# apache/datafusion-ballista

Measured on NVIDIA B200. Metric: tpch_q1_rows_per_sec, higher is better.
Workload: dtype decimal128/i128

## Files before the change

### datafusion-ballista_b200/csrc/device/kernels.cu

```cuda
#include <cuda_runtime.h>
#include <stdint.h>

#include "../common/hash.hpp"
#include "../common/tpch_gen.hpp"
#include "kernels.h"

namespace b200 {

typedef __int128 i128;
typedef unsigned __int128 u128;

static inline int grid_for(int64_t n, int block, int per_thread = 1) {
  int64_t g = (n + (int64_t)block * per_thread - 1) / ((int64_t)block * per_thread);
  if (g < 1) g = 1;
  if (g > 148 * 16) g = 148 * 16;
  return (int)g;
}

__global__ void agg_table_init_kernel(AggTable T, AccKinds kinds) {
  for (unsigned long long i = blockIdx.x * (unsigned long long)blockDim.x + threadIdx.x; i < T.cap; i += (unsigned long long)gridDim.x * blockDim.x) {
    T.hash[i] = 0;
    T.state[i] = 0;
    T.lock[i] = 0;
    for (int a = 0; a < kinds.n; a++) {
// ... 26 lines not shown
    case PH_I8:
    case PH_U8:
    case PH_BOOL8: ((int8_t*)data)[pos] = (int8_t)v; break;
    case PH_I16:
    case PH_U16: ((int16_t*)data)[pos] = (int16_t)v; break;
    case PH_I32:
    case PH_U32: ((int32_t*)data)[pos] = (int32_t)v; break;
    default: ((long long*)data)[pos] = v;
  }
}

__global__ void agg_extract_kernel(AggTable T, AggExtractArgs A) {
  for (unsigned long long s = blockIdx.x * (unsigned long long)blockDim.x + threadIdx.x; s < T.cap; s += (unsigned long long)gridDim.x * blockDim.x) {
    if (T.state[s] != 2) continue;
    unsigned long long pos = atomicAdd(A.counter, 1ull);
    for (int j = 0; j < A.n_out; j++) {
      const AggOut& o = A.out[j];
      switch (o.kind) {
        case AO_KEY: {
          unsigned long long w0 = T.keys[((unsigned long long)o.a * T.cap + s) * 2 + 0];
          unsigned long long w1 = T.keys[((unsigned long long)o.a * T.cap + s) * 2 + 1];
          unsigned char v = T.key_valid[(unsigned long long)o.a * T.cap + s];
          if (o.phys == PH_DEC128 || o.phys == PH_STRVIEW) ((ulonglong2*)o.data)[pos] = make_ulonglong2(w0, w1);
          else if (o.phys == PH_F64) ((unsigned long long*)o.data)[pos] = w0;
          else if (o.phys == PH_F32) ((float*)o.data)[pos] = (float)__longlong_as_double((long long)w0);
          else store_typed_i64(o.data, o.phys, pos, (long long)w0);
          if (o.valid) o.valid[pos] = v;
          break;
        }
        case AO_KEY_PACKED: {
// ... 786 lines not shown
```

### datafusion-ballista_b200/csrc/device/kernels.h

```cpp
#pragma once
#include <cuda_runtime.h>
#include <stdint.h>

#include "program.h"

namespace b200 {

cudaError_t launch_pipeline(const Program& P, int reg_groups, int grid, int block, size_t smem, cudaStream_t st);
cudaError_t launch_fused_pipeline(const Program& P, const FusedSpec& F, FusedShape shape, int reg_groups, int grid, int block, size_t smem, cudaStream_t st,
                                  int* is_static);
bool fused_rows_ok(const Program& P, int grid, int block, int rows_per_thread);
bool pipeline_add_only(const Program& P, int grid, int block);

struct AccKinds {
  uint8_t kind[VM_MAX_ACC];
  int n;
};
void launch_agg_table_init(const AggTable& T, const AccKinds& kinds, cudaStream_t st);

enum AggOutKind : uint8_t {
  AO_KEY = 0,
  AO_ACC_I128,
  AO_ACC_I64,
  AO_ACC_F64,
// ... 5 lines not shown
};
struct AggOut {
  void* data;
  uint8_t* valid;
  void* aux;
  uint8_t kind;
  uint8_t a, b;
  uint8_t phys;
  int32_t imm;
};
struct AggExtractArgs {
  AggOut out[VM_MAX_OUT];
  int n_out;
  int n_keys;
  unsigned long long* counter;
  unsigned int* error;
};
void launch_agg_extract(const AggTable& T, const AggExtractArgs& A, cudaStream_t st);

void launch_scan_u32_to_u64(const uint32_t* in, uint64_t* out, int64_t n, uint64_t* scratch , cudaStream_t st);
void launch_histogram_u32(const uint32_t* ids, int64_t n, uint32_t n_bins, unsigned long long* counts, cudaStream_t st);
uint64_t launch_partition_dest_stable(const uint32_t* ids, int64_t n, uint32_t n_bins, uint32_t* dest, uint64_t* keys_a, uint32_t* vals_a, uint64_t* keys_b,
                                      uint32_t* vals_b, uint32_t* hist_scratch, uint64_t* scan_scratch, cudaStream_t st);
void launch_scatter_fixed(const void* in, void* out, const uint32_t* dest, int64_t n, int width, cudaStream_t st);
void launch_gather_fixed(const void* in, const uint8_t* valid_in, void* out, uint8_t* valid_out, const int64_t* idx, int64_t n, int width, cudaStream_t st);
static const int GATHER_MAX_COLS = 32;
struct GatherCol {
  const void* in;
  const uint8_t* valid_in;
  void* out;
// ... 212 lines not shown
```

### datafusion-ballista_b200/csrc/host/engine.cpp

```cpp
#include <sched.h>
#include <sys/stat.h>

#include <algorithm>
#include <atomic>
#include <cctype>
#include <chrono>
#include <cmath>
#include <cstdio>
#include <map>
#include <mutex>
#include <functional>
#include <set>

#include "../common/arrow_host.hpp"
#include "../common/tpch_gen.hpp"
#include "../device/kernels.h"
#include "host_pool.hpp"
#include "lower.hpp"
#include "nccl_dyn.hpp"
#include "../common/plan_proto.hpp"
#include "../common/plan_dump.hpp"
#include "parquet_meta.hpp"
#include "arrow_ipc.hpp"

// ... 34 lines not shown
  int sm_count = 148;
  cudaStream_t own_stream = nullptr;
  cudaStream_t stream = nullptr;
  std::mutex mu;
  std::map<std::string, std::map<int, DevBatchPtr>> tables;
  std::map<ShuffleKey, std::vector<Piece>> shuffle;
  std::map<ShuffleKey, DevBatchPtr> packed_cache;
  std::atomic<uint64_t> launches{0};
  std::atomic<uint64_t> n_fused{0}, n_fused_static{0}, n_vm{0}, n_groupby{0}, n_groupby_pf{0}, n_fastfilter{0};
  int64_t batch_size = 8192;
  std::map<std::string, std::string> config;
  std::map<std::string, int> agg_hint;
  uint64_t pf_bucket_slots = (uint64_t)1 << 19;
  int64_t pf_min_rows = (int64_t)1 << 22;
  std::map<std::string, uint64_t> agg_groups;
  void* pinned_stage = nullptr;
  std::unique_ptr<HostPool> pool;
  std::mutex ingest_mu;
  struct NarrowSlot {
    void* pinned = nullptr;
    void* dev = nullptr;
    cudaEvent_t done = nullptr;
    bool used = false;
    size_t bytes = 0;
  } nslot[4];
  int64_t ingest_chunk_rows = (int64_t)1 << 22;
  int ingest_slots = 3;
  bool kernel_timing = false;
  struct KernelSample { std::string name; cudaEvent_t e0, e1; uint64_t bytes; };
  std::vector<KernelSample> ksamples;
  struct KernelStat { double ms = 0; uint64_t launches = 0, bytes = 0; };
  std::map<std::string, KernelStat> kstats;
  ncclComm_t comm = nullptr;
  std::mutex comm_mu;
  uint64_t exch_sent_bytes = 0, exch_recv_bytes = 0;
  size_t win_config_bytes = 0;
  uint8_t* win_local = nullptr;
  size_t win_bytes = 0, win_used = 0;
  std::vector<uint8_t*> win_peer;
  uint64_t fused_exchanges = 0;
  std::mutex export_mu;
  uint8_t* export_arena = nullptr;
  std::atomic<uint64_t> narrowed_bytes_saved{0};
};

struct b200_stage {
  b200_engine* eng = nullptr;
  std::string job_id;
  int64_t stage_id = 0;
  PlanPtr plan;
  std::string fingerprint;
  std::vector<OpMetrics> metrics;
  std::map<const PlanNode*, int> metric_index;
};

#define NCCL_CHECK(expr)                                                                                              \
  do {                                                                                                                \
    ncclResult_t _r = (expr);                                                                                         \
    if (_r != 0) throw EngineError(B200_ERR_CUDA, std::string("NCCL error: ") + NcclApi::get().GetErrorString(_r) + " at " + __FILE__ + ":" + std::to_string(__LINE__)); \
  } while (0)

static void release_window(b200_engine* e);
static void setup_window(b200_engine* e);

namespace {

struct TaskCtx {
  uint8_t* arena = nullptr;
  size_t pos = 0;
  bool drained = true;
  std::vector<std::function<void()>> checks;
};
static const size_t TASK_ARENA_BYTES = (size_t)1 << 16;
inline TaskCtx& task_ctx() {
  static thread_local TaskCtx t;
  if (!t.arena && cudaHostAlloc((void**)&t.arena, TASK_ARENA_BYTES, cudaHostAllocDefault) != cudaSuccess) t.arena = nullptr;
  return t;
}

struct Exec {
  b200_engine* e;
  b200_stage* s;
  const volatile int32_t* cancel;
  cudaStream_t st() const { return e->stream; }
  void check_cancel() const {
    if (cancel && *cancel) throw EngineError(B200_ERR_CANCELLED, "task cancelled");
  }
  void count(uint64_t n = 1) const { e->launches.fetch_add(n, std::memory_order_relaxed); }
  OpMetrics* m(const PlanNode* n) const {
    if (!s) return nullptr;
    auto it = s->metric_index.find(n);
    return it == s->metric_index.end() ? nullptr : &s->metrics[(size_t)it->second];
  }
  const void* fetch_bytes(const void* dptr, size_t bytes) const {
    TaskCtx& t = task_ctx();
    if (!t.arena) throw EngineError(B200_ERR_OOM, "pinned read-back arena unavailable");
    if (t.drained) {
      t.pos = 0;
// ... 21 lines not shown
      t.pos = 0;
      t.drained = false;
      at = 0;
      if (bytes > TASK_ARENA_BYTES) throw EngineError(B200_ERR_INVALID, "staging request larger than the arena");
    }
    t.pos = at + bytes;
    return t.arena + at;
  }
  template <class T>
  const T* fetch(const void* dptr) const {
    return (const T*)fetch_bytes(dptr, sizeof(T));
  }
  void defer(std::function<void()> fn) const { task_ctx().checks.push_back(std::move(fn)); }
  void sync() const {
    TaskCtx& t = task_ctx();
    cudaError_t se = cudaStreamSynchronize(st());
    t.drained = true;
    std::vector<std::function<void()>> cs;
    cs.swap(t.checks);
    CUDA_CHECK(se);
    for (auto& c : cs) c();
    check_cancel();
  }
  static void abandon() {
    TaskCtx& t = task_ctx();
    t.checks.clear();
    t.drained = true;
  }
  template <class T>
  T get(const void* dptr) const {
    const T* p = fetch<T>(dptr);
    sync();
    return *p;
  }
};

struct KernelTimer {
// ... 526 lines not shown
      CUDA_CHECK(cudaMemsetAsync(cnt->ptr, 0, 8, st));
      launch_bytes_to_bitmap(c.valid, (uint8_t*)bm->ptr, n, (unsigned long long*)cnt->ptr, st);
      x.count();
      h.validity.resize((size_t)(n + 7) / 8);
      CUDA_CHECK(cudaMemcpyAsync(h.validity.data(), bm->ptr, h.validity.size(), cudaMemcpyDeviceToHost, st));
      h.null_count = (int64_t)x.get<unsigned long long>(cnt->ptr);
      if (h.null_count == 0) h.validity.clear();
    }
    if (c.type.id == TypeId::Bool) {
      h.data.assign((size_t)(n + 7) / 8, 0);
      if (n) {
        DevPtr bm = dev_alloc((size_t)(n + 7) / 8 + 16, st);
        launch_bytes_to_bitmap(c.data, (uint8_t*)bm->ptr, n, nullptr, st);
        x.count();
        CUDA_CHECK(cudaMemcpyAsync(h.data.data(), bm->ptr, h.data.size(), cudaMemcpyDeviceToHost, st));
        CUDA_CHECK(cudaStreamSynchronize(st));
      }
    } else if (c.type.id == TypeId::Utf8) {
      DevColumn u = c.phys == PH_STRVIEW ? as_utf8(x, c) : c;
      h.data.resize((size_t)(n + 1) * 4);
      CUDA_CHECK(cudaMemcpyAsync(h.data.data(), u.data, h.data.size(), cudaMemcpyDeviceToHost, st));
      CUDA_CHECK(cudaStreamSynchronize(st));
      int32_t* off = (int32_t*)h.data.data();
      int32_t first = off[0], last = off[n];
      h.extra.resize((size_t)(last - first));
      if (last > first) CUDA_CHECK(cudaMemcpyAsync(h.extra.data(), u.chars + first, h.extra.size(), cudaMemcpyDeviceToHost, st));
      CUDA_CHECK(cudaStreamSynchronize(st));
      for (int64_t i = 0; i <= n; i++) off[i] -= first;
    } else {
      h.data.resize((size_t)n * c.width());
      if (n) CUDA_CHECK(cudaMemcpyAsync(h.data.data(), c.data, h.data.size(), cudaMemcpyDeviceToHost, st));
      CUDA_CHECK(cudaStreamSynchronize(st));
    }
    hcs.push_back(std::move(h));
  }
  return hcs;
}

void export_batch(const Exec& x, const DevBatch& b, int64_t r0, int64_t r1, ArrowArray* out, ArrowSchema* out_schema) {
  std::vector<HostCol> hcs = download_batch(x, b, r0, r1);
  export_record_batch(std::move(hcs), r1 - r0, out, out_schema);
}

struct RunOutcome {
  RunStatus status;
  float ms = 0;
};

struct FusedPlan {
  FusedSpec spec;
  FusedShape shape;
  int block = 0;
  size_t smem = 0;
};

static void throw_run_error(unsigned int error) {
  if (error == 1) throw EngineError(B200_ERR_EXECUTION, "Arithmetic overflow");
  if (error == 2) throw EngineError(B200_ERR_EXECUTION, "Divide by zero");
  if (error) throw EngineError(B200_ERR_EXECUTION, "execution error in expression");
}

// ... 156 lines not shown
  CUDA_CHECK(cudaEventRecord(e1, x.st()));
  x.count();
  RunOutcome o;
  const RunStatus* hs = x.fetch<RunStatus>(dstat->ptr);
  const unsigned int* he = extra_fetch ? x.fetch<unsigned int>(extra_fetch) : nullptr;
  if (!wait) {
    x.defer([hs, e0, e1, met, dstat, tstate]() {
      float ms = 0;
      cudaEventElapsedTime(&ms, e0, e1);
      cudaEventDestroy(e0);
      cudaEventDestroy(e1);
      if (met) met->elapsed_ns += (uint64_t)(ms * 1e6);
      throw_run_error(hs->error);
    });
    memset(&o.status, 0, sizeof o.status);
    return o;
  }
  try {
    x.sync();
  } catch (...) {
    cudaEventDestroy(e0);
    cudaEventDestroy(e1);
    throw;
  }
  o.status = *hs;
  if (he && extra_out) *extra_out = *he;
  cudaEventElapsedTime(&o.ms, e0, e1);
  cudaEventDestroy(e0);
  cudaEventDestroy(e1);
  if (met) met->elapsed_ns += (uint64_t)(o.ms * 1e6);
// ... 719 lines not shown
    S.out_data[j] = oc.data;
  }
  S.n_out = P.n_out;
  S.n_rows = P.n_rows;
  return true;
}

struct TableMem {
  AggTable T;
  std::vector<DevPtr> keep;
};

TableMem alloc_table(const Exec& x, uint64_t cap, int n_keys, const std::vector<AccDesc>& accs) {
  TableMem tm;
  memset(&tm.T, 0, sizeof tm.T);
  auto A = [&](size_t bytes) {
    DevPtr p = dev_alloc(bytes, x.st());
    tm.keep.push_back(p);
    return p->ptr;
  };
  tm.T.cap = cap;
  tm.T.hash = (unsigned long long*)A(cap * 8);
  tm.T.state = (unsigned int*)A(cap * 4);
  tm.T.lock = (unsigned int*)A(cap * 4);
  tm.T.keys = (unsigned long long*)A(std::max<size_t>(1, (size_t)n_keys) * cap * 16);
  tm.T.key_valid = (unsigned char*)A(std::max<size_t>(1, (size_t)n_keys) * cap);
  tm.T.acc = (unsigned long long*)A(std::max<size_t>(1, accs.size()) * cap * 16);
  tm.T.n_groups = (unsigned int*)A(16);
  AccKinds k;
  memset(&k, 0, sizeof k);
  k.n = (int)accs.size();
  for (size_t i = 0; i < accs.size(); i++) k.kind[i] = accs[i].kind;
  launch_agg_table_init(tm.T, k, x.st());
  x.count();
  return tm;
}

typedef std::function<std::unique_ptr<PipelineBuilder>()> BuilderFactory;

DevBatchPtr run_aggregate(const Exec& x, const BuilderFactory& make_pb, const PlanNode& node, const DevBatchPtr& src, OpMetrics* met) {
  const int n_keys = (int)node.group_by.size();
  if (n_keys > VM_MAX_KEYS) throw EngineError(B200_ERR_UNSUPPORTED, "too many group-by columns");
  int pack_mode = 0;
  {
    bool any_str = false, all_narrow = n_keys > 0;
    for (auto& g : node.group_by) {
      any_str |= g.expr->type.id == TypeId::Utf8;
      all_narrow &= narrowable(g.expr->type);
    }
    if (n_keys == 2 && all_narrow) pack_mode = 2;
    else if (any_str) pack_mode = 1;
  }
  int node_idx = -1;
  if (x.s) {
    auto it = x.s->metric_index.find(&node);
    if (it != x.s->metric_index.end()) node_idx = it->second;
  }
  const std::string hint_key = (x.s ? x.s->fingerprint : std::string("?")) + "#" + std::to_string(node_idx);
  int level = 0;
  bool had_hint = false;
  uint64_t groups_hint = 0;
  {
    std::lock_guard<std::mutex> g(x.e->mu);
    auto it = x.e->agg_hint.find(hint_key);
    if (it != x.e->agg_hint.end()) {
      level = it->second / 4;
      pack_mode = std::min(pack_mode, it->second % 4);
      had_hint = true;
      auto ig = x.e->agg_groups.find(hint_key);
      if (ig != x.e->agg_groups.end()) groups_hint = ig->second;
    }
  }
  const int hinted_level = had_hint ? level : -1;
  bool sampled = false;
  std::unique_ptr<PipelineBuilder> pbp;
  AggLowered L;
  TableMem tm;
  RunOutcome ro;
  unsigned int n_groups = 0;
  bool gb_bailed = false, pf_off = false;
  for (;;) {
    x.check_cancel();
    ScopeTimer t_iter("  agg: lower+alloc+launch+sync");
    pbp = make_pb();
    PipelineBuilder& pb = *pbp;
    L = AggLowered();
    lower_aggregate(pb, node, L, pack_mode);
    Program& P = pb.prog;
    P.n_keys = (uint8_t)n_keys;
    P.n_acc = (uint8_t)L.accs.size();
    for (int k = 0; k < n_keys; k++) P.keys[k] = pb.resolve(L.keys[(size_t)k]);
    for (size_t a = 0; a < L.accs.size(); a++) P.acc[a] = L.accs[a];
    memset(&P.key_hash, 0, sizeof P.key_hash);
    P.keys_all_i64 = L.fast ? 1 : 0;
    if (n_keys) {
      if (L.fast) {
// ... 45 lines not shown
        RunOutcome so = launch_program(x, pb, 0, nullptr, true, nullptr, stm.T.n_groups, &seen, &probe);
        if (!so.status.pack_overflow && (so.status.overflow || seen > (unsigned)VM_REG_GROUPS)) {
          level = (so.status.overflow || (int64_t)seen * 2 > sample_rows) ? 3 : 2;
          continue;
        }
      }
      P.table = tm.T;
    }
    FusedPlan fspec;
    const bool use_fused = level == 0 && match_fused(P, fspec);
    GroupBySpec gspec;
    const bool use_gb = level > 0 && !gb_bailed && match_groupby(P, gspec);
    gspec.pf_K = pf_off ? -1 : 0;
    {
      ScopeTimer t_l("    agg: launch_program (incl. sync)");
      ro = launch_program(x, pb, reg_groups, use_fused ? &fspec : nullptr, true, met, tm.T.n_groups, &n_groups, use_gb ? &gspec : nullptr);
    }
    if (met) met->launches += 2;
    if (ro.status.pack_overflow && use_gb) {
      gb_bailed = true;
      continue;
    }
    if (ro.status.pack_overflow) {
      pack_mode = pack_mode == 2 ? 1 : 0;
      continue;
    }
    if (!ro.status.overflow) break;
    if (level > 0 && cap >= next_pow2((uint64_t)std::max<int64_t>(src->n, 1) * 2)) {
      if (use_gb && !pf_off) {
        pf_off = true;
        continue;
      }
      throw EngineError(B200_ERR_EXECUTION, "aggregate hash table overflow");
    }
    level++;
  }
  {
    int learnt = level;
    if (level > 0) {
      learnt = 1;
      while (learnt < 7 && ((uint64_t)1 << (12 + 4 * learnt)) < (uint64_t)n_groups * 2) learnt++;
    }
    std::lock_guard<std::mutex> g(x.e->mu);
    x.e->agg_hint[hint_key] = learnt * 4 + pack_mode;
    uint64_t& gh = x.e->agg_groups[hint_key];
    gh = std::max<uint64_t>(gh, n_groups);
  }
  PipelineBuilder& pb = *pbp;
  ScopeTimer t_ex("  agg: extract");
  auto out = std::make_shared<DevBatch>();
  out->n = n_groups;
  AggExtractArgs A;
  memset(&A, 0, sizeof A);
  if (L.outs.size() > (size_t)VM_MAX_OUT) throw EngineError(B200_ERR_UNSUPPORTED, "too many aggregate output columns");
  A.n_out = (int)L.outs.size();
  A.n_keys = n_keys;
  DevPtr counter = dev_alloc(16, x.st());
  CUDA_CHECK(cudaMemsetAsync(counter->ptr, 0, 16, x.st()));
  A.counter = (unsigned long long*)counter->ptr;
  A.error = (unsigned int*)((uint8_t*)counter->ptr + 8);
  uint64_t wbytes = 0;
  for (size_t j = 0; j < L.outs.size(); j++) {
    const auto& r = L.outs[j];
    DevColumn oc = make_out_column(r.name, r.type, r.phys, n_groups, r.with_valid, x.st());
    oc.n = n_groups;
    if (r.key_idx >= 0) {
      for (auto& k : L.keys[(size_t)r.key_idx].keep) oc.keep.push_back(k);
      if (r.phys == PH_STRVIEW) {
        for (auto& sc : src->cols)
          for (auto& k : sc.keep) oc.keep.push_back(k);
        for (auto& k : pb.keep) oc.keep.push_back(k);
      }
    }
    AggOut& o = A.out[j];
    o.data = (void*)oc.data;
    o.valid = (uint8_t*)oc.valid;
    o.aux = nullptr;
    if (r.kind == AO_KEY_PACKED) {
      DevPtr ch = dev_alloc((size_t)std::max<unsigned int>(n_groups, 1) * 8, x.st());
      o.aux = ch->ptr;
      oc.keep.push_back(ch);
    }
    o.kind = r.kind;
    o.a = r.a;
    o.b = r.b;
    o.phys = r.phys;
    o.imm = r.imm;
    wbytes += (uint64_t)oc.width() * n_groups;
    out->cols.push_back(oc);
  }
  launch_agg_extract(tm.T, A, x.st());
  x.count();
  {
    const unsigned int* herr = x.fetch<unsigned int>(A.error);
    x.defer([herr, counter]() {
      if (*herr) throw EngineError(B200_ERR_EXECUTION, "Arithmetic overflow");
    });
  }
  for (size_t c = 0; c < out->cols.size() && c < node.schema.size(); c++) out->cols[c].name = node.schema[c].name;
  if (met) {
    met->bytes_read += source_bytes(pb);
    met->bytes_written += wbytes;
    met->input_rows += (uint64_t)src->n;
  }
  return out;
}

struct Runner {
  Exec x;
  std::string job;
// ... 7 lines not shown
        return it->second.empty() ? 0 : it->second.rbegin()->first + 1;
      }
      case PlanNode::ShuffleReader: {
        std::lock_guard<std::mutex> g(x.e->mu);
        int mx = 0;
        for (auto& kv : x.e->shuffle)
          if (kv.first.job == job && kv.first.stage == n.reader_stage_id) mx = std::max(mx, (int)kv.first.part + 1);
        return mx;
      }
      case PlanNode::SortPreservingMerge: return 1;
      case PlanNode::Passthrough:
        if (n.op_name == "CoalescePartitionsExec") return 1;
        return n_partitions(*n.children[0]);
      case PlanNode::HashJoin: return n_partitions(*n.children[1]);
      default: return n_partitions(*n.children[0]);
    }
  }

  DevBatchPtr concat(const std::vector<DevBatchPtr>& parts, const Schema& schema) {
    std::vector<std::pair<DevBatchPtr, std::pair<int64_t, int64_t>>> v;
    for (auto& p : parts) v.push_back({p, {0, p->n}});
    return concat_slices(v, schema);
  }

  DevBatchPtr concat_slices(const std::vector<std::pair<DevBatchPtr, std::pair<int64_t, int64_t>>>& parts, const Schema& schema) {
    auto out = std::make_shared<DevBatch>();
    int64_t total = 0;
    for (auto& p : parts) total += p.second.second - p.second.first;
    out->n = total;
    if (parts.size() == 1) {
// ... 179 lines not shown
          const int64_t keep = std::min<int64_t>(all->n, n.fetch);
          out = std::make_shared<DevBatch>();
          out->n = keep;
          for (auto& c : all->cols) out->cols.push_back(slice_column(c, 0, keep));
          break;
        }
        out = with_chain(n, part, false, [&](const BuilderFactory& mk, DevBatchPtr& src) {
          auto pb = mk();
          return run_materialize(x, *pb, named_cols(*pb, n.schema), src, met);
        });
        break;
      }
      case PlanNode::Aggregate: {
        const PlanNode& child = *n.children[0];
        bool all = (n.agg_mode == AggMode::Final || n.agg_mode == AggMode::Single) && part == 0 && n_partitions(child) > 1;
        out = with_chain(child, part, all, [&](const BuilderFactory& mk, DevBatchPtr& src) { return run_aggregate(x, mk, n, src, met); });
        break;
      }
      case PlanNode::HashJoin:
        out = exec_join(n, part, met);
        if (!n.sort_keys.empty()) out = do_sort(n.sort_keys, -1, out, met);
        break;
      case PlanNode::Sort: {
        DevBatchPtr in = exec(*n.children[0], part);
        out = do_sort(n.sort_keys, n.fetch, in, met);
        break;
      }
      case PlanNode::SortPreservingMerge: {
        DevBatchPtr in = exec_all(*n.children[0]);
        out = do_sort(n.sort_keys, n.fetch, in, met);
        break;
      }
      case PlanNode::Passthrough:
        out = (n.op_name == "CoalescePartitionsExec") ? exec_all(*n.children[0]) : exec(*n.children[0], part);
        break;
      case PlanNode::Limit: {
        DevBatchPtr in = (n.op_name == "GlobalLimitExec") ? exec_all(*n.children[0]) : exec(*n.children[0], part);
        int64_t r0 = std::min<int64_t>(std::max<int64_t>(0, n.skip), in->n);
        int64_t r1 = n.fetch >= 0 ? std::min<int64_t>(in->n, r0 + n.fetch) : in->n;
        out = std::make_shared<DevBatch>();
        out->n = r1 - r0;
        for (auto& c : in->cols) out->cols.push_back(slice_column(c, r0, r1));
        break;
      }
// ... 103 lines not shown
          radix_sort_pairs_u64((uint64_t*)ka->ptr, (uint32_t*)vb->ptr, (uint64_t*)kb->ptr, (uint32_t*)va->ptr, n, (uint32_t*)hist->ptr, (uint64_t*)scan->ptr, x.st(), &in_a, &ln);
          perm = in_a ? (uint32_t*)vb->ptr : (uint32_t*)va->ptr;
        }
        x.count(ln);
        (void)perm_alt;
      }
    }
    int64_t m = fetch >= 0 ? std::min<int64_t>(fetch, n) : n;
    DevPtr idx = dev_alloc((size_t)std::max<int64_t>(m, 1) * 8, x.st());
    launch_u32_to_i64(perm, (int64_t*)idx->ptr, m, x.st());
    x.count();
    DevBatch proj;
    proj.n = n;
    for (size_t c = 0; c < n_in_cols; c++) proj.cols.push_back(in->cols[c]);
    DevBatchPtr out = gather_batch(x, proj, (const int64_t*)idx->ptr, m, false);
    CUDA_CHECK(cudaStreamSynchronize(x.st()));
    if (met) {
      met->elapsed_ns += (uint64_t)std::chrono::duration_cast<std::chrono::nanoseconds>(std::chrono::steady_clock::now() - t0).count();
      met->input_rows += (uint64_t)n;
    }
    return out;
  }

  struct Mixed {
    std::vector<DevColumn> cols;
    int64_t n = 0;
  };
  Mixed materialize_mixed(PipelineBuilder& pb, const std::vector<ColRef>& outs, const DevBatchPtr& src, OpMetrics* met) {
    Mixed m;
    const bool filters = program_filters(pb.prog);
    std::vector<int> direct(outs.size(), -1);
// ... 309 lines not shown
  }

  uint64_t slice_bytes(const DevBatch& b, int64_t rows, const std::vector<int64_t>& chars_bytes) {
    uint64_t t = 0;
    size_t si = 0;
    for (auto& c : b.cols) {
      if (c.type.id == TypeId::Bool) t += (uint64_t)(rows + 7) / 8;
      else if (c.type.id == TypeId::Utf8) t += 4ull * (uint64_t)(rows + 1) + (uint64_t)chars_bytes[si++];
      else t += (uint64_t)c.width() * (uint64_t)rows;
    }
    return t;
  }

  std::vector<int64_t> string_bytes(const DevBatch& b) {
    std::vector<int64_t> out;
    PartStrCols sc;
    sc.n = 0;
    std::vector<size_t> unknown;
    for (auto& c : b.cols) {
      if (c.type.id != TypeId::Utf8) continue;
      if (c.phys == PH_UTF8 && c.chars_bytes >= 0) {
        out.push_back(c.chars_bytes);
        continue;
      }
      out.push_back(-1);
      if (b.n == 0) {
        out.back() = 0;
        continue;
      }
      if (sc.n == PART_MAX_STR_COLS) throw EngineError(B200_ERR_UNSUPPORTED, "more than 16 string columns in one shuffle output");
      sc.c[sc.n++] = PartStrCol{c.data, c.valid, c.phys == PH_STRVIEW ? 1 : 0, 0};
      unknown.push_back(out.size() - 1);
    }
    if (sc.n) {
      DevPtr acc = dev_alloc((size_t)(1 + sc.n) * 8, x.st());
      CUDA_CHECK(cudaMemsetAsync(acc->ptr, 0, (size_t)(1 + sc.n) * 8, x.st()));
      PidSrc none;
      memset(&none, 0, sizeof none);
      CUDA_CHECK(launch_partition_hist(none, b.n, 1, nullptr, (unsigned long long*)acc->ptr, sc, (unsigned long long*)acc->ptr + 1, x.st()));
      x.count();
      const unsigned long long* h = (const unsigned long long*)x.fetch_bytes((const unsigned long long*)acc->ptr + 1, (size_t)sc.n * 8);
      x.sync();
      for (size_t k = 0; k < unknown.size(); k++) out[unknown[k]] = (int64_t)h[k];
    }
    return out;
  }

  struct FusedExchange {
    bool done = false;
    uint64_t sent = 0, recvd = 0;
  };

  bool scatter_to_owners(const PlanNode& root, int input_partition, const std::vector<DevColumn>& pay, const PidSrc& pid, int64_t n, uint32_t P,
                         uint32_t n_tiles, const DevPtr& mat, const DevPtr& tile_hist, uint64_t row_bytes, FusedExchange* fx,
                         std::vector<b200_shuffle_write_partition>& res, OpMetrics* met) {
    b200_engine* e = x.e;
    NcclApi& N = NcclApi::get();
    const int W = e->world, me = e->rank;
    const size_t mrow = (size_t)P + 3;
    const size_t ncols = pay.size();
// ... 186 lines not shown
    auto nbatches = [&](uint64_t rows) { return (rows + (uint64_t)bs - 1) / (uint64_t)bs; };
    std::vector<b200_shuffle_write_partition> res;
    const bool single = root.n_out_partitions == 1;
    if (root.n_out_partitions == 0 || single) {
      DevBatchPtr in = exec(child, input_partition);
      auto st = std::make_shared<DevBatch>();
      st->n = in->n;
      for (size_t c = 0; c < in->cols.size(); c++) {
        DevColumn col = in->cols[c];
        col.name = root.schema[c].name;
        st->cols.push_back(col);
      }
      std::vector<int64_t> cb;
      {
        ScopeTimer t2("writer: string bytes + final sync");
        cb = string_bytes(*st);
        x.sync();
      }
      b200_shuffle_write_partition w{};
      w.partition_id = single ? 0u : (uint64_t)input_partition;
      w.num_rows = (uint64_t)st->n;
      w.num_batches = nbatches(w.num_rows);
      w.num_bytes = slice_bytes(*st, st->n, cb);
      w.file_id = single ? (int64_t)input_partition : -1;
      w.is_sort_shuffle = (single && root.sort_shuffle) ? 1 : 0;
      {
        std::lock_guard<std::mutex> g(x.e->mu);
        auto& v = x.e->shuffle[ShuffleKey{job, root.stage_id, single ? 0 : input_partition}];
        if (single) {
          const int64_t fid = (int64_t)input_partition;
          v.erase(std::remove_if(v.begin(), v.end(), [&](const Piece& pc) { return pc.file_id == fid && pc.src_rank == my_rank; }), v.end());
// ... 979 lines not shown
    cudaMemPool_t pool;
    CUDA_CHECK(cudaDeviceGetDefaultMemPool(&pool, device));
    uint64_t thr = pool_bytes ? pool_bytes : UINT64_MAX;
    CUDA_CHECK(cudaMemPoolSetAttribute(pool, cudaMemPoolAttrReleaseThreshold, &thr));
    *out = e;
  });
}

void b200_engine_destroy(b200_engine* e) {
  if (!e) return;
  cudaSetDevice(e->device);
  cudaStreamSynchronize(e->stream);
  e->tables.clear();
  e->shuffle.clear();
  e->packed_cache.clear();
  cudaStreamSynchronize(e->stream);
  for (auto& sl : e->nslot) {
    if (sl.pinned) cudaFreeHost(sl.pinned);
    if (sl.dev) cudaFree(sl.dev);
    if (sl.done) cudaEventDestroy(sl.done);
  }
  release_window(e);
  if (e->comm && NcclApi::get().ok()) NcclApi::get().CommDestroy(e->comm);
  if (e->export_arena) cudaFreeHost(e->export_arena);
  if (e->own_stream) cudaStreamDestroy(e->own_stream);
  delete e;
}

int b200_engine_set_stream(b200_engine* e, void* cuda_stream) {
  return guard([&] {
// ... 7 lines not shown
    CUDA_CHECK(cudaStreamSynchronize(e->stream));
  });
}
uint64_t b200_engine_kernel_launches(b200_engine* e) { return e->launches; }
uint64_t b200_engine_counter(b200_engine* e, const char* name) {
  const std::string n = name ? name : "";
  if (n == "fused") return e->n_fused;
  if (n == "groupby_partition_first") return e->n_groupby_pf;
  if (n == "fused_static") return e->n_fused_static;
  if (n == "fused_exchanges") return e->fused_exchanges;
  if (n == "exchange_window_bytes") return e->win_bytes;
  if (n == "vm") return e->n_vm;
  if (n == "groupby") return e->n_groupby;
  if (n == "fastfilter") return e->n_fastfilter;
  if (n == "ingest_bytes_saved") return e->narrowed_bytes_saved;
  return 0;
}

int b200_engine_set_config(b200_engine* e, const char* key, const char* value) {
  return guard([&] {
    std::lock_guard<std::mutex> g(e->mu);
    e->config[key] = value;
    if (std::string(key) == "datafusion.execution.batch_size") e->batch_size = std::max<int64_t>(1, atoll(value));
    if (std::string(key) == "b200.ingest.chunk_rows") e->ingest_chunk_rows = std::max<int64_t>(1 << 16, atoll(value));
    if (std::string(key) == "b200.ingest.slots") e->ingest_slots = atoi(value);
    if (std::string(key) == "b200.exchange.window_bytes") e->win_config_bytes = (size_t)strtoull(value, nullptr, 10);
    if (std::string(key) == "b200.ingest.threads") e->pool.reset();
    if (std::string(key) == "b200.agg.partition_first.bucket_slots") {
      const uint64_t v = strtoull(value, nullptr, 10);
      e->pf_bucket_slots = v ? std::max<uint64_t>(next_pow2(v), 64) : 0;
    }
    if (std::string(key) == "b200.agg.partition_first.min_rows") e->pf_min_rows = std::max<int64_t>(1, atoll(value));
    if (std::string(key) == "b200.agg.reset_hints") {
      e->agg_hint.clear();
      e->agg_groups.clear();
    }
    if (std::string(key) == "b200.metrics.kernel_timing") e->kernel_timing = std::string(value) == "on" || std::string(value) == "1" || std::string(value) == "true";
  });
}

int b200_engine_register_batch(b200_engine* e, const char* table, int partition, struct ArrowArray* batch, struct ArrowSchema* schema) {
  return guard([&] {
    CUDA_CHECK(cudaSetDevice(e->device));
    DevBatchPtr b = import_batch(e, batch, schema);
    Exec x{e, nullptr, nullptr};
    prepack_short_strings(x, *b);
    DevBatchPtr prev;
    {
      std::lock_guard<std::mutex> g(e->mu);
      auto& slot = e->tables[table][partition];
// ... 193 lines not shown
    {
      std::lock_guard<std::mutex> g(e->mu);
      auto it = e->tables.find(table);
      if (it == e->tables.end() || !it->second.count(partition)) throw EngineError(B200_ERR_NOT_FOUND, "no such table partition");
      b = it->second[partition];
    }
    Exec x{e, nullptr, nullptr};
    export_batch(x, *b, 0, b->n, out, out_schema);
  });
}

int b200_stage_prepare(b200_engine* e, const char* job_id, int64_t stage_id, const char* plan_json, uint64_t plan_len, b200_stage** out) {
  ScopeTimer tm("stage_prepare");
  return guard([&] {
    if (!e || !plan_json || !out) throw EngineError(B200_ERR_INVALID, "null argument");
    Json j = parse_json(plan_json, plan_len ? (size_t)plan_len : strlen(plan_json));
    PlanPtr plan = parse_plan(j);
    if (plan->op != PlanNode::ShuffleWriter)
      throw EngineError(B200_ERR_INVALID, "Plan passed to new_query_stage_exec is not a ShuffleWriterExec");
    auto* s = new b200_stage();
    s->eng = e;
    s->job_id = job_id ? job_id : plan->job_id;
    s->stage_id = stage_id;
    plan->stage_id = stage_id;
    {
      std::string shape(plan_json, plan_len ? (size_t)plan_len : strlen(plan_json));
      const std::string tag = "\"job_id\":\"";
      size_t at = shape.find(tag);
      if (at != std::string::npos) {
        size_t end = shape.find('"', at + tag.size());
        if (end != std::string::npos) shape.erase(at + tag.size(), end - at - tag.size());
      }
      s->fingerprint = std::to_string(stage_id) + ":" + std::to_string(mix64(hash_bytes((const uint8_t*)shape.data(), (uint32_t)shape.size())));
    }
    collect_nodes(*plan, s);
    s->plan = std::move(plan);
    *out = s;
  });
}

int b200_plan_proto_to_json(const void* plan_bytes, uint64_t n_bytes, const char* job_id, char** out_json) {
  return guard([&] {
    if (!plan_bytes || !out_json) throw EngineError(B200_ERR_INVALID, "null argument");
    std::string js;
    try {
      js = pbp::plan_proto_to_json(plan_bytes, (size_t)n_bytes, job_id ? std::string(job_id) : std::string());
    } catch (const pbp::Unsupported& u) {
      throw EngineError(B200_ERR_UNSUPPORTED, u.what());
    } catch (const std::runtime_error& r) {
// ... 133 lines not shown
    }
    char* m = (char*)malloc(w.out.size() + 1);
    if (!m) throw EngineError(B200_ERR_OOM, "task status");
    memcpy(m, w.out.data(), w.out.size());
    m[w.out.size()] = 0;
    *out_bytes = m;
    *out_len = w.out.size();
  });
}

int b200_stage_execute(b200_stage* s, int input_partition, const volatile int32_t* cancel_flag, b200_shuffle_write_partition* out, int cap, int* n_out) {
  ScopeTimer tm("stage_execute");
  return guard([&] {
    if (!s || !n_out) throw EngineError(B200_ERR_INVALID, "null argument");
    CUDA_CHECK(cudaSetDevice(s->eng->device));
    Exec x{s->eng, s, cancel_flag};
    Runner r{x, s->job_id};
    std::vector<b200_shuffle_write_partition> res;
    try {
      res = r.execute_stage(*s->plan, input_partition);
    } catch (...) {
      cudaStreamSynchronize(s->eng->stream);
      Exec::abandon();
      {
        std::lock_guard<std::mutex> g(s->eng->mu);
        for (auto it = s->eng->shuffle.begin(); it != s->eng->shuffle.end();) {
          if (it->first.job == s->job_id && it->first.stage == s->stage_id) {
            auto& v = it->second;
            v.erase(std::remove_if(v.begin(), v.end(), [&](const Piece& pc) { return (pc.file_id == input_partition || (pc.file_id < 0 && it->first.part == input_partition)) && pc.src_rank == s->eng->rank; }), v.end());
            if (v.empty()) {
              it = s->eng->shuffle.erase(it);
              continue;
            }
          }
          ++it;
        }
      }
      throw;
    }
    if ((int)res.size() > cap) throw EngineError(B200_ERR_INVALID, "output array too small");
    for (size_t i = 0; i < res.size(); i++) out[i] = res[i];
    *n_out = (int)res.size();
  });
}

int b200_stage_execute_exchange(b200_stage* s, int input_partition, const volatile int32_t* cancel_flag, b200_shuffle_write_partition* out, int cap,
                                int* n_out, b200_exchange_stats* stats) {
  ScopeTimer tm("stage_execute_exchange");
  return guard([&] {
    if (!s || !n_out) throw EngineError(B200_ERR_INVALID, "null argument");
    b200_engine* e = s->eng;
    if (s->plan->op != PlanNode::ShuffleWriter || s->plan->n_out_partitions < 1)
// ... 2 lines not shown
    Exec x{e, s, cancel_flag};
    Runner r{x, s->job_id};
    Runner::FusedExchange fx;
    std::vector<b200_shuffle_write_partition> res;
    uint64_t sent = 0, recvd = 0;
    try {
      res = r.execute_stage(*s->plan, input_partition, &fx);
      if (fx.done) {
        sent = fx.sent;
        recvd = fx.recvd;
      } else if (e->world > 1) {
        Exchange ex{x, Runner{x, s->job_id}, e, s->job_id, s->stage_id, (int)s->plan->n_out_partitions, EXCH_HASH, 0, s->plan->schema, s->plan->schema.size()};
        ex.run(&sent, &recvd);
      }
    } catch (...) {
      cudaStreamSynchronize(e->stream);
      Exec::abandon();
      throw;
    }
    e->exch_sent_bytes += sent;
    e->exch_recv_bytes += recvd;
    if (stats) {
      stats->sent_bytes = sent;
      stats->recv_bytes = recvd;
    }
    if ((int)res.size() > cap) throw EngineError(B200_ERR_INVALID, "output array too small");
    for (size_t i = 0; i < res.size(); i++) out[i] = res[i];
    *n_out = (int)res.size();
  });
}
// ... 547 lines not shown
```

Baseline: 38.32 billion.

## Speculate aggregate group counts, cache parsed plans, and coalesce agg allocations

Adds several host-side latency cuts. Aggregates reuse the group count from an earlier run of the same stage and partition, so the launch no longer needs a blocking sync. The check is deferred, and a mismatch throws and re-executes the stage without speculation. Parsed plans are cached by a job-agnostic fingerprint. Hash-table and extract-output buffers now come from single allocations, with a memset replacing the init kernel where possible. Single-run SortPreservingMerge skips the sort, and string-byte counting defers its sync. The risks are re-execution cost on a miss, a shared cached plan, and extra bookkeeping.

```diff
diff --git a/datafusion-ballista_b200/csrc/device/kernels.cu b/datafusion-ballista_b200/csrc/device/kernels.cu
--- a/datafusion-ballista_b200/csrc/device/kernels.cu
+++ b/datafusion-ballista_b200/csrc/device/kernels.cu
@@ -64,6 +64,7 @@
   for (unsigned long long s = blockIdx.x * (unsigned long long)blockDim.x + threadIdx.x; s < T.cap; s += (unsigned long long)gridDim.x * blockDim.x) {
     if (T.state[s] != 2) continue;
     unsigned long long pos = atomicAdd(A.counter, 1ull);
+    if (pos >= A.cap) continue;
     for (int j = 0; j < A.n_out; j++) {
       const AggOut& o = A.out[j];
       switch (o.kind) {
diff --git a/datafusion-ballista_b200/csrc/device/kernels.h b/datafusion-ballista_b200/csrc/device/kernels.h
--- a/datafusion-ballista_b200/csrc/device/kernels.h
+++ b/datafusion-ballista_b200/csrc/device/kernels.h
@@ -43,6 +43,7 @@
   int n_out;
   int n_keys;
   unsigned long long* counter;
+  unsigned long long cap;
   unsigned int* error;
 };
 void launch_agg_extract(const AggTable& T, const AggExtractArgs& A, cudaStream_t st);
diff --git a/datafusion-ballista_b200/csrc/host/engine.cpp b/datafusion-ballista_b200/csrc/host/engine.cpp
--- a/datafusion-ballista_b200/csrc/host/engine.cpp
+++ b/datafusion-ballista_b200/csrc/host/engine.cpp
@@ -72,6 +72,7 @@
   uint64_t pf_bucket_slots = (uint64_t)1 << 19;
   int64_t pf_min_rows = (int64_t)1 << 22;
   std::map<std::string, uint64_t> agg_groups;
+  std::map<std::string, uint64_t> agg_spec;
   void* pinned_stage = nullptr;
   std::unique_ptr<HostPool> pool;
   std::mutex ingest_mu;
@@ -100,13 +101,18 @@
   std::mutex export_mu;
   uint8_t* export_arena = nullptr;
   std::atomic<uint64_t> narrowed_bytes_saved{0};
+  std::atomic<uint64_t> stream_syncs{0};
+  struct CachedPlan { std::shared_ptr<const PlanNode> plan; uint64_t used; };
+  std::map<std::string, CachedPlan> plan_cache;
+  uint64_t plan_cache_tick = 0;
 };
+static const size_t PLAN_CACHE_ENTRIES = 32;
 
 struct b200_stage {
   b200_engine* eng = nullptr;
   std::string job_id;
   int64_t stage_id = 0;
-  PlanPtr plan;
+  std::shared_ptr<const PlanNode> plan;
   std::string fingerprint;
   std::vector<OpMetrics> metrics;
   std::map<const PlanNode*, int> metric_index;
@@ -136,10 +142,13 @@
   return t;
 }
 
+struct SpeculationMiss {};
+
 struct Exec {
   b200_engine* e;
   b200_stage* s;
   const volatile int32_t* cancel;
+  bool speculate = false;
   cudaStream_t st() const { return e->stream; }
   void check_cancel() const {
     if (cancel && *cancel) throw EngineError(B200_ERR_CANCELLED, "task cancelled");
@@ -191,6 +200,7 @@
   void defer(std::function<void()> fn) const { task_ctx().checks.push_back(std::move(fn)); }
   void sync() const {
     TaskCtx& t = task_ctx();
+    e->stream_syncs++;
     cudaError_t se = cudaStreamSynchronize(st());
     t.drained = true;
     std::vector<std::function<void()>> cs;
@@ -198,6 +208,10 @@
     CUDA_CHECK(se);
     for (auto& c : cs) c();
     check_cancel();
+  }
+  void wait() const {
+    e->stream_syncs++;
+    CUDA_CHECK(cudaStreamSynchronize(st()));
   }
   static void abandon() {
     TaskCtx& t = task_ctx();
@@ -754,23 +768,23 @@
         launch_bytes_to_bitmap(c.data, (uint8_t*)bm->ptr, n, nullptr, st);
         x.count();
         CUDA_CHECK(cudaMemcpyAsync(h.data.data(), bm->ptr, h.data.size(), cudaMemcpyDeviceToHost, st));
-        CUDA_CHECK(cudaStreamSynchronize(st));
+        x.wait();
       }
     } else if (c.type.id == TypeId::Utf8) {
       DevColumn u = c.phys == PH_STRVIEW ? as_utf8(x, c) : c;
       h.data.resize((size_t)(n + 1) * 4);
       CUDA_CHECK(cudaMemcpyAsync(h.data.data(), u.data, h.data.size(), cudaMemcpyDeviceToHost, st));
-      CUDA_CHECK(cudaStreamSynchronize(st));
+      x.wait();
       int32_t* off = (int32_t*)h.data.data();
       int32_t first = off[0], last = off[n];
       h.extra.resize((size_t)(last - first));
       if (last > first) CUDA_CHECK(cudaMemcpyAsync(h.extra.data(), u.chars + first, h.extra.size(), cudaMemcpyDeviceToHost, st));
-      CUDA_CHECK(cudaStreamSynchronize(st));
+      x.wait();
       for (int64_t i = 0; i <= n; i++) off[i] -= first;
     } else {
       h.data.resize((size_t)n * c.width());
       if (n) CUDA_CHECK(cudaMemcpyAsync(h.data.data(), c.data, h.data.size(), cudaMemcpyDeviceToHost, st));
-      CUDA_CHECK(cudaStreamSynchronize(st));
+      x.wait();
     }
     hcs.push_back(std::move(h));
   }
@@ -785,6 +799,8 @@
 struct RunOutcome {
   RunStatus status;
   float ms = 0;
+  const RunStatus* deferred = nullptr;
+  const unsigned int* deferred_extra = nullptr;
 };
 
 struct FusedPlan {
@@ -971,6 +987,8 @@
       throw_run_error(hs->error);
     });
     memset(&o.status, 0, sizeof o.status);
+    o.deferred = hs;
+    o.deferred_extra = he;
     return o;
   }
   try {
@@ -1720,31 +1738,43 @@
 TableMem alloc_table(const Exec& x, uint64_t cap, int n_keys, const std::vector<AccDesc>& accs) {
   TableMem tm;
   memset(&tm.T, 0, sizeof tm.T);
-  auto A = [&](size_t bytes) {
-    DevPtr p = dev_alloc(bytes, x.st());
-    tm.keep.push_back(p);
-    return p->ptr;
-  };
+  auto up = [](size_t b) { return (b + 255) & ~(size_t)255; };
+  const size_t nk = std::max<size_t>(1, (size_t)n_keys), na = std::max<size_t>(1, accs.size());
+  const size_t o_hash = 256, o_state = o_hash + up(cap * 8), o_lock = o_state + up(cap * 4), o_acc = o_lock + up(cap * 4);
+  const size_t o_keys = o_acc + up(na * cap * 16), o_kv = o_keys + up(nk * cap * 16), bytes = o_kv + up(nk * cap);
+  DevPtr blk = dev_alloc(bytes, x.st());
+  tm.keep.push_back(blk);
+  uint8_t* const b = (uint8_t*)blk->ptr;
   tm.T.cap = cap;
-  tm.T.hash = (unsigned long long*)A(cap * 8);
-  tm.T.state = (unsigned int*)A(cap * 4);
-  tm.T.lock = (unsigned int*)A(cap * 4);
-  tm.T.keys = (unsigned long long*)A(std::max<size_t>(1, (size_t)n_keys) * cap * 16);
-  tm.T.key_valid = (unsigned char*)A(std::max<size_t>(1, (size_t)n_keys) * cap);
-  tm.T.acc = (unsigned long long*)A(std::max<size_t>(1, accs.size()) * cap * 16);
-  tm.T.n_groups = (unsigned int*)A(16);
+  tm.T.n_groups = (unsigned int*)b;
+  tm.T.hash = (unsigned long long*)(b + o_hash);
+  tm.T.state = (unsigned int*)(b + o_state);
+  tm.T.lock = (unsigned int*)(b + o_lock);
+  tm.T.acc = (unsigned long long*)(b + o_acc);
+  tm.T.keys = (unsigned long long*)(b + o_keys);
+  tm.T.key_valid = (unsigned char*)(b + o_kv);
   AccKinds k;
   memset(&k, 0, sizeof k);
   k.n = (int)accs.size();
-  for (size_t i = 0; i < accs.size(); i++) k.kind[i] = accs[i].kind;
-  launch_agg_table_init(tm.T, k, x.st());
-  x.count();
+  bool zero_init = true;
+  for (size_t i = 0; i < accs.size(); i++) {
+    k.kind[i] = accs[i].kind;
+    zero_init &= accs[i].kind != ACC_MIN_I128 && accs[i].kind != ACC_MAX_I128 && accs[i].kind != ACC_MIN_F64 && accs[i].kind != ACC_MAX_F64;
+  }
+  if (zero_init) {
+    CUDA_CHECK(cudaMemsetAsync(b, 0, o_keys, x.st()));
+  } else {
+    launch_agg_table_init(tm.T, k, x.st());
+    x.count();
+  }
   return tm;
 }
 
 typedef std::function<std::unique_ptr<PipelineBuilder>()> BuilderFactory;
 
-DevBatchPtr run_aggregate(const Exec& x, const BuilderFactory& make_pb, const PlanNode& node, const DevBatchPtr& src, OpMetrics* met) {
+static const uint64_t SPEC_MAX_GROUPS = 4096;
+
+DevBatchPtr run_aggregate(const Exec& x, const BuilderFactory& make_pb, const PlanNode& node, const DevBatchPtr& src, OpMetrics* met, int part) {
   const int n_keys = (int)node.group_by.size();
   if (n_keys > VM_MAX_KEYS) throw EngineError(B200_ERR_UNSUPPORTED, "too many group-by columns");
   int pack_mode = 0;
@@ -1763,9 +1793,12 @@
     if (it != x.s->metric_index.end()) node_idx = it->second;
   }
   const std::string hint_key = (x.s ? x.s->fingerprint : std::string("?")) + "#" + std::to_string(node_idx);
+  const std::string spec_key = hint_key + "@" + std::to_string(part);
   int level = 0;
   bool had_hint = false;
   uint64_t groups_hint = 0;
+  bool speculate = false;
+  uint64_t spec_groups = 0;
   {
     std::lock_guard<std::mutex> g(x.e->mu);
     auto it = x.e->agg_hint.find(hint_key);
@@ -1775,6 +1808,11 @@
       had_hint = true;
       auto ig = x.e->agg_groups.find(hint_key);
       if (ig != x.e->agg_groups.end()) groups_hint = ig->second;
+      auto is = x.e->agg_spec.find(spec_key);
+      if (x.speculate && is != x.e->agg_spec.end()) {
+        speculate = true;
+        spec_groups = is->second;
+      }
     }
   }
   const int hinted_level = had_hint ? level : -1;
@@ -1785,7 +1823,9 @@
   RunOutcome ro;
   unsigned int n_groups = 0;
   bool gb_bailed = false, pf_off = false;
+  int attempts = 0;
   for (;;) {
+    attempts++;
     x.check_cancel();
     ScopeTimer t_iter("  agg: lower+alloc+launch+sync");
     pbp = make_pb();
@@ -1861,9 +1901,18 @@
     gspec.pf_K = pf_off ? -1 : 0;
     {
       ScopeTimer t_l("    agg: launch_program (incl. sync)");
-      ro = launch_program(x, pb, reg_groups, use_fused ? &fspec : nullptr, true, met, tm.T.n_groups, &n_groups, use_gb ? &gspec : nullptr);
+      ro = launch_program(x, pb, reg_groups, use_fused ? &fspec : nullptr, !speculate, met, tm.T.n_groups, &n_groups, use_gb ? &gspec : nullptr);
     }
     if (met) met->launches += 2;
+    if (speculate) {
+      const RunStatus* hs = ro.deferred;
+      const unsigned int* hg = ro.deferred_extra;
+      x.defer([hs, hg, spec_groups]() {
+        if (hs->overflow || hs->pack_overflow || *hg != spec_groups) throw SpeculationMiss();
+      });
+      n_groups = (unsigned int)spec_groups;
+      break;
+    }
     if (ro.status.pack_overflow && use_gb) {
       gb_bailed = true;
       continue;
@@ -1882,7 +1931,7 @@
     }
     level++;
   }
-  {
+  if (!speculate) {
     int learnt = level;
     if (level > 0) {
       learnt = 1;
@@ -1892,6 +1941,8 @@
     x.e->agg_hint[hint_key] = learnt * 4 + pack_mode;
     uint64_t& gh = x.e->agg_groups[hint_key];
     gh = std::max<uint64_t>(gh, n_groups);
+    if (attempts == 1 && n_groups <= SPEC_MAX_GROUPS) x.e->agg_spec[spec_key] = n_groups;
+    else x.e->agg_spec.erase(spec_key);
   }
   PipelineBuilder& pb = *pbp;
   ScopeTimer t_ex("  agg: extract");
@@ -1902,15 +1953,42 @@
   if (L.outs.size() > (size_t)VM_MAX_OUT) throw EngineError(B200_ERR_UNSUPPORTED, "too many aggregate output columns");
   A.n_out = (int)L.outs.size();
   A.n_keys = n_keys;
-  DevPtr counter = dev_alloc(16, x.st());
-  CUDA_CHECK(cudaMemsetAsync(counter->ptr, 0, 16, x.st()));
-  A.counter = (unsigned long long*)counter->ptr;
-  A.error = (unsigned int*)((uint8_t*)counter->ptr + 8);
+  const size_t rows = std::max<unsigned int>(n_groups, 1);
+  auto up = [](size_t b) { return (b + 255) & ~(size_t)255; };
+  struct Place { size_t data = 0, valid = 0, aux = 0; };
+  std::vector<Place> place(L.outs.size());
+  size_t blk_bytes = 256;
+  for (size_t j = 0; j < L.outs.size(); j++) {
+    const auto& r = L.outs[j];
+    place[j].data = blk_bytes;
+    blk_bytes += up(rows * phys_width(r.phys));
+    if (r.with_valid) {
+      place[j].valid = blk_bytes;
+      blk_bytes += up(rows);
+    }
+    if (r.kind == AO_KEY_PACKED) {
+      place[j].aux = blk_bytes;
+      blk_bytes += up(rows * 8);
+    }
+  }
+  DevPtr blk = dev_alloc(blk_bytes, x.st());
+  uint8_t* const base = (uint8_t*)blk->ptr;
+  CUDA_CHECK(cudaMemsetAsync(base, 0, speculate ? blk_bytes : 16, x.st()));
+  A.counter = (unsigned long long*)base;
+  A.error = (unsigned int*)(base + 8);
+  A.cap = n_groups;
   uint64_t wbytes = 0;
   for (size_t j = 0; j < L.outs.size(); j++) {
     const auto& r = L.outs[j];
-    DevColumn oc = make_out_column(r.name, r.type, r.phys, n_groups, r.with_valid, x.st());
+    DevColumn oc;
+    oc.name = r.name;
+    oc.type = r.type;
+    oc.phys = r.phys;
     oc.n = n_groups;
+    oc.data = base + place[j].data;
+    if (r.with_valid) oc.valid = base + place[j].valid;
+    oc.nullable = r.with_valid;
+    oc.keep.push_back(blk);
     if (r.key_idx >= 0) {
       for (auto& k : L.keys[(size_t)r.key_idx].keep) oc.keep.push_back(k);
       if (r.phys == PH_STRVIEW) {
@@ -1922,12 +2000,7 @@
     AggOut& o = A.out[j];
     o.data = (void*)oc.data;
     o.valid = (uint8_t*)oc.valid;
-    o.aux = nullptr;
-    if (r.kind == AO_KEY_PACKED) {
-      DevPtr ch = dev_alloc((size_t)std::max<unsigned int>(n_groups, 1) * 8, x.st());
-      o.aux = ch->ptr;
-      oc.keep.push_back(ch);
-    }
+    o.aux = r.kind == AO_KEY_PACKED ? base + place[j].aux : nullptr;
     o.kind = r.kind;
     o.a = r.a;
     o.b = r.b;
@@ -1940,7 +2013,7 @@
   x.count();
   {
     const unsigned int* herr = x.fetch<unsigned int>(A.error);
-    x.defer([herr, counter]() {
+    x.defer([herr, blk]() {
       if (*herr) throw EngineError(B200_ERR_EXECUTION, "Arithmetic overflow");
     });
   }
@@ -1978,6 +2051,26 @@
         return n_partitions(*n.children[0]);
       case PlanNode::HashJoin: return n_partitions(*n.children[1]);
       default: return n_partitions(*n.children[0]);
+    }
+  }
+
+  bool one_run(const PlanNode& n) {
+    switch (n.op) {
+      case PlanNode::ShuffleReader: {
+        std::lock_guard<std::mutex> g(x.e->mu);
+        auto it = x.e->shuffle.find(ShuffleKey{job, n.reader_stage_id, 0});
+        int pieces = 0;
+        if (it != x.e->shuffle.end())
+          for (auto& p : it->second) pieces += p.r1 > p.r0 ? 1 : 0;
+        return pieces <= 1;
+      }
+      case PlanNode::Passthrough:
+        if (n.op_name == "CoalescePartitionsExec" && n_partitions(*n.children[0]) != 1) return false;
+        return one_run(*n.children[0]);
+      case PlanNode::Filter:
+      case PlanNode::Projection:
+      case PlanNode::Limit: return one_run(*n.children[0]);
+      default: return true;
     }
   }
 
@@ -2187,7 +2280,7 @@
       case PlanNode::Aggregate: {
         const PlanNode& child = *n.children[0];
         bool all = (n.agg_mode == AggMode::Final || n.agg_mode == AggMode::Single) && part == 0 && n_partitions(child) > 1;
-        out = with_chain(child, part, all, [&](const BuilderFactory& mk, DevBatchPtr& src) { return run_aggregate(x, mk, n, src, met); });
+        out = with_chain(child, part, all, [&](const BuilderFactory& mk, DevBatchPtr& src) { return run_aggregate(x, mk, n, src, met, part); });
         break;
       }
       case PlanNode::HashJoin:
@@ -2200,7 +2293,21 @@
         break;
       }
       case PlanNode::SortPreservingMerge: {
-        DevBatchPtr in = exec_all(*n.children[0]);
+        const PlanNode& child = *n.children[0];
+        if (n_partitions(child) == 1 && one_run(child)) {
+          DevBatchPtr in = exec(child, 0);
+          if (met) met->input_rows += (uint64_t)in->n;
+          const int64_t m = n.fetch >= 0 ? std::min<int64_t>(n.fetch, in->n) : in->n;
+          if (m == in->n) {
+            out = in;
+            break;
+          }
+          out = std::make_shared<DevBatch>();
+          out->n = m;
+          for (auto& c : in->cols) out->cols.push_back(slice_column(c, 0, m));
+          break;
+        }
+        DevBatchPtr in = exec_all(child);
         out = do_sort(n.sort_keys, n.fetch, in, met);
         break;
       }
@@ -2334,7 +2441,7 @@
     proj.n = n;
     for (size_t c = 0; c < n_in_cols; c++) proj.cols.push_back(in->cols[c]);
     DevBatchPtr out = gather_batch(x, proj, (const int64_t*)idx->ptr, m, false);
-    CUDA_CHECK(cudaStreamSynchronize(x.st()));
+    x.wait();
     if (met) {
       met->elapsed_ns += (uint64_t)std::chrono::duration_cast<std::chrono::nanoseconds>(std::chrono::steady_clock::now() - t0).count();
       met->input_rows += (uint64_t)n;
@@ -2674,6 +2781,11 @@
 
   std::vector<int64_t> string_bytes(const DevBatch& b) {
     std::vector<int64_t> out;
+    queue_string_bytes(b, out);
+    x.sync();
+    return out;
+  }
+  void queue_string_bytes(const DevBatch& b, std::vector<int64_t>& out) {
     PartStrCols sc;
     sc.n = 0;
     std::vector<size_t> unknown;
@@ -2700,10 +2812,10 @@
       CUDA_CHECK(launch_partition_hist(none, b.n, 1, nullptr, (unsigned long long*)acc->ptr, sc, (unsigned long long*)acc->ptr + 1, x.st()));
       x.count();
       const unsigned long long* h = (const unsigned long long*)x.fetch_bytes((const unsigned long long*)acc->ptr + 1, (size_t)sc.n * 8);
-      x.sync();
-      for (size_t k = 0; k < unknown.size(); k++) out[unknown[k]] = (int64_t)h[k];
-    }
-    return out;
+      x.defer([h, unknown, &out]() {
+        for (size_t k = 0; k < unknown.size(); k++) out[unknown[k]] = (int64_t)h[k];
+      });
+    }
   }
 
   struct FusedExchange {
@@ -2920,7 +3032,7 @@
       std::vector<int64_t> cb;
       {
         ScopeTimer t2("writer: string bytes + final sync");
-        cb = string_bytes(*st);
+        queue_string_bytes(*st, cb);
         x.sync();
       }
       b200_shuffle_write_partition w{};
@@ -3930,6 +4042,7 @@
   e->tables.clear();
   e->shuffle.clear();
   e->packed_cache.clear();
+  e->plan_cache.clear();
   cudaStreamSynchronize(e->stream);
   for (auto& sl : e->nslot) {
     if (sl.pinned) cudaFreeHost(sl.pinned);
@@ -3967,6 +4080,7 @@
   if (n == "groupby") return e->n_groupby;
   if (n == "fastfilter") return e->n_fastfilter;
   if (n == "ingest_bytes_saved") return e->narrowed_bytes_saved;
+  if (n == "stream_syncs") return e->stream_syncs;
   return 0;
 }
 
@@ -3987,6 +4101,7 @@
     if (std::string(key) == "b200.agg.reset_hints") {
       e->agg_hint.clear();
       e->agg_groups.clear();
+      e->agg_spec.clear();
     }
     if (std::string(key) == "b200.metrics.kernel_timing") e->kernel_timing = std::string(value) == "on" || std::string(value) == "1" || std::string(value) == "true";
   });
@@ -4210,25 +4325,45 @@
   ScopeTimer tm("stage_prepare");
   return guard([&] {
     if (!e || !plan_json || !out) throw EngineError(B200_ERR_INVALID, "null argument");
-    Json j = parse_json(plan_json, plan_len ? (size_t)plan_len : strlen(plan_json));
-    PlanPtr plan = parse_plan(j);
-    if (plan->op != PlanNode::ShuffleWriter)
-      throw EngineError(B200_ERR_INVALID, "Plan passed to new_query_stage_exec is not a ShuffleWriterExec");
+    const size_t len = plan_len ? (size_t)plan_len : strlen(plan_json);
+    std::string shape(plan_json, len);
+    const std::string tag = "\"job_id\":\"";
+    size_t at = shape.find(tag);
+    if (at != std::string::npos) {
+      size_t end = shape.find('"', at + tag.size());
+      if (end != std::string::npos) shape.erase(at + tag.size(), end - at - tag.size());
+    }
+    const std::string stage_tag = std::to_string(stage_id) + ":";
+    const std::string key = stage_tag + (job_id ? shape : std::string(plan_json, len));
+    std::shared_ptr<const PlanNode> plan;
+    {
+      std::lock_guard<std::mutex> g(e->mu);
+      auto it = e->plan_cache.find(key);
+      if (it != e->plan_cache.end()) {
+        it->second.used = ++e->plan_cache_tick;
+        plan = it->second.plan;
+      }
+    }
+    if (!plan) {
+      PlanPtr parsed = parse_plan(parse_json(plan_json, len));
+      if (parsed->op != PlanNode::ShuffleWriter)
+        throw EngineError(B200_ERR_INVALID, "Plan passed to new_query_stage_exec is not a ShuffleWriterExec");
+      parsed->stage_id = stage_id;
+      plan = std::shared_ptr<const PlanNode>(std::move(parsed));
+      std::lock_guard<std::mutex> g(e->mu);
+      if (e->plan_cache.size() >= PLAN_CACHE_ENTRIES) {
+        auto lru = e->plan_cache.begin();
+        for (auto it = e->plan_cache.begin(); it != e->plan_cache.end(); ++it)
+          if (it->second.used < lru->second.used) lru = it;
+        e->plan_cache.erase(lru);
+      }
+      e->plan_cache[key] = b200_engine::CachedPlan{plan, ++e->plan_cache_tick};
+    }
     auto* s = new b200_stage();
     s->eng = e;
     s->job_id = job_id ? job_id : plan->job_id;
     s->stage_id = stage_id;
-    plan->stage_id = stage_id;
-    {
-      std::string shape(plan_json, plan_len ? (size_t)plan_len : strlen(plan_json));
-      const std::string tag = "\"job_id\":\"";
-      size_t at = shape.find(tag);
-      if (at != std::string::npos) {
-        size_t end = shape.find('"', at + tag.size());
-        if (end != std::string::npos) shape.erase(at + tag.size(), end - at - tag.size());
-      }
-      s->fingerprint = std::to_string(stage_id) + ":" + std::to_string(mix64(hash_bytes((const uint8_t*)shape.data(), (uint32_t)shape.size())));
-    }
+    s->fingerprint = stage_tag + std::to_string(mix64(hash_bytes((const uint8_t*)shape.data(), (uint32_t)shape.size())));
     collect_nodes(*plan, s);
     s->plan = std::move(plan);
     *out = s;
@@ -4392,28 +4527,37 @@
   return guard([&] {
     if (!s || !n_out) throw EngineError(B200_ERR_INVALID, "null argument");
     CUDA_CHECK(cudaSetDevice(s->eng->device));
-    Exec x{s->eng, s, cancel_flag};
-    Runner r{x, s->job_id};
     std::vector<b200_shuffle_write_partition> res;
-    try {
-      res = r.execute_stage(*s->plan, input_partition);
-    } catch (...) {
+    auto discard = [&]() {
+      s->eng->stream_syncs++;
       cudaStreamSynchronize(s->eng->stream);
       Exec::abandon();
-      {
-        std::lock_guard<std::mutex> g(s->eng->mu);
-        for (auto it = s->eng->shuffle.begin(); it != s->eng->shuffle.end();) {
-          if (it->first.job == s->job_id && it->first.stage == s->stage_id) {
-            auto& v = it->second;
-            v.erase(std::remove_if(v.begin(), v.end(), [&](const Piece& pc) { return (pc.file_id == input_partition || (pc.file_id < 0 && it->first.part == input_partition)) && pc.src_rank == s->eng->rank; }), v.end());
-            if (v.empty()) {
-              it = s->eng->shuffle.erase(it);
-              continue;
-            }
+      std::lock_guard<std::mutex> g(s->eng->mu);
+      for (auto it = s->eng->shuffle.begin(); it != s->eng->shuffle.end();) {
+        if (it->first.job == s->job_id && it->first.stage == s->stage_id) {
+          auto& v = it->second;
+          v.erase(std::remove_if(v.begin(), v.end(), [&](const Piece& pc) { return (pc.file_id == input_partition || (pc.file_id < 0 && it->first.part == input_partition)) && pc.src_rank == s->eng->rank; }), v.end());
+          if (v.empty()) {
+            it = s->eng->shuffle.erase(it);
+            continue;
           }
-          ++it;
-        }
-      }
+        }
+        ++it;
+      }
+    };
+    const std::vector<OpMetrics> metrics0 = s->metrics;
+    try {
+      try {
+        Runner r{Exec{s->eng, s, cancel_flag, true}, s->job_id};
+        res = r.execute_stage(*s->plan, input_partition);
+      } catch (const SpeculationMiss&) {
+        discard();
+        s->metrics = metrics0;
+        Runner r{Exec{s->eng, s, cancel_flag, false}, s->job_id};
+        res = r.execute_stage(*s->plan, input_partition);
+      }
+    } catch (...) {
+      discard();
       throw;
     }
     if ((int)res.size() > cap) throw EngineError(B200_ERR_INVALID, "output array too small");
@@ -4446,6 +4590,7 @@
         ex.run(&sent, &recvd);
       }
     } catch (...) {
+      e->stream_syncs++;
       cudaStreamSynchronize(e->stream);
       Exec::abandon();
       throw;
```

After: 41.95 billion, median of 6. 9.5% higher.
